# zdebruine/singlet

Hardware: AMD Instinct MI355X
Metric: ALS iterations/sec (1M cells x 30k genes, 5% nnz, k=50) (higher is better)
Workload: dtype f64

## Files before the change

singlet_amd/csrc/kernels_tiled.hip:

```cpp
#include "sgl_internal.h"
#include <atomic>
#include <hipcub/hipcub.hpp>
#include <stdlib.h>
#include <utility>
#include <type_traits>

#define TILED_NW 8
#define TILED_CW 64
#define TILED_NP 32
#define TILED_LDS_BYTES (160 * 1024 - 512)
#define TILED_SLACK 4096

__device__ __forceinline__ int64_t tiled_slot_col(const int32_t* __restrict__ perm, int64_t ncol, int64_t wb, int h, int p, int nsl) {
    const int64_t pos = wb * (TILED_NP * nsl) + nsl * p + h;
    if (pos >= ncol) return -1;
    return perm ? (int64_t)perm[pos] : pos;
}

__global__ void tiled_count_kernel(const int64_t* __restrict__ seg, const int32_t* __restrict__ perm, int64_t ncol, int T, int64_t nwb,
                                   uint8_t* __restrict__ cnt, int64_t* __restrict__ chunk_entries, int nsl) {
    const int64_t u = (int64_t)blockIdx.x * blockDim.x + threadIdx.x;
    if (u >= nwb * T) return;
    const int64_t wb = u / T;
    const int t = (int)(u - wb * T);
    int64_t tot = 0;
    for (int p = 0; p < TILED_NP; ++p) {
        int64_t n = 0;
        for (int h = 0; h < nsl; ++h) {
            const int64_t col = tiled_slot_col(perm, ncol, wb, h, p, nsl);
            if (col >= 0) {
                const int64_t c = seg[(int64_t)(t + 1) * ncol + col] - seg[(int64_t)t * ncol + col];
                n = c > n ? c : n;
            }
        }
        int g = (int)((n + 3) >> 2);
        const int gps = 16 / nsl;
        if (p == TILED_NP - 1) g += (int)((gps - ((tot + g) & (gps - 1))) & (gps - 1));
        cnt[u * TILED_NP + p] = (uint8_t)g;
        tot += g;
    }
    chunk_entries[u] = tot * 4 * nsl;
}

__global__ __launch_bounds__(256) void tiled_fill_kernel(const double* __restrict__ x, const int32_t* __restrict__ idx,
                                                         const int64_t* __restrict__ seg, const int32_t* __restrict__ perm,
                                                         int64_t ncol, int T, int64_t nwb, int TR, int row_bytes,
                                                         const uint8_t* __restrict__ cnt,
                                                         const int64_t* __restrict__ cstart,
                                                         uint32_t* __restrict__ sroff, double* __restrict__ sx,
                                                         int masked, uint64_t seed, SglDiv inv_density, int mask_t,
                                                         int64_t col_off, int64_t row_off, int nsl) {
    const int lane = threadIdx.x & 63;
    const int eps = 64 / nsl, eps_sh = nsl == 4 ? 4 : 5;
    const int64_t gw = ((int64_t)blockIdx.x * blockDim.x + threadIdx.x) >> 6;
    const int64_t nw = ((int64_t)gridDim.x * blockDim.x) >> 6;
    for (int64_t u = gw; u < nwb * T; u += nw) {
        const int64_t wb = u / T;
        const int t = (int)(u - wb * T);
        const int64_t c0 = cstart[u];
        int P = 0;
        for (int p = 0; p < TILED_NP; ++p) {
            const int n4 = 4 * (int)cnt[u * TILED_NP + p];
            if (n4 == 0) continue;
            for (int h = 0; h < nsl; ++h) {
                const int64_t col = tiled_slot_col(perm, ncol, wb, h, p, nsl);
                int64_t a = 0, b = 0;
                if (col >= 0) { a = seg[(int64_t)t * ncol + col]; b = seg[(int64_t)(t + 1) * ncol + col]; }
                for (int q = lane; q < n4; q += 64) {
                    uint32_t ro = 0;
                    double xv = 0.0;
                    if (a + q < b) {
                        const int32_t r = idx[a + q];
                        ro = (uint32_t)(r - t * TR) * (uint32_t)row_bytes;
                        xv = x[a + q];
                        if (masked) {
                            const uint64_t gc = (uint64_t)(col + col_off), gr = (uint64_t)(r + row_off);
                            if (mask_t ? sgl_draw(seed, gr, gc, inv_density) : sgl_draw(seed, gc, gr, inv_density)) xv = 0.0;
                        }
                    }
                    const int pos = P + q;
                    const int64_t dst = c0 + (int64_t)(pos >> eps_sh) * 64 + h * eps + (pos & (eps - 1));
                    if (sroff != nullptr) sroff[dst] = ro;
                    sx[dst] = xv;
                }
            }
            P += n4;
        }
    }
// ... 34 lines not shown
    *p = nullptr;
    *cap = 0;
    const size_t want = count + count / 32 + 64;
    SGLCHK(t_alloc(p, want));
    *cap = want;
    return SGL_OK;
}

void sgl_tiled_free(DevTiled& S) {
    if (S.seg) (void)sgl_pool_free(S.seg);
    if (S.perm) (void)sgl_pool_free(S.perm);
    if (S.roff) (void)sgl_pool_free(S.roff);
    if (S.x) (void)sgl_pool_free(S.x);
    if (S.cstart) (void)sgl_pool_free(S.cstart);
    if (S.cnt) (void)sgl_pool_free(S.cnt);
    if (S.gtab) (void)sgl_pool_free(S.gtab);
    if (S.part) (void)sgl_pool_free(S.part);
    if (S.xm) (void)sgl_pool_free(S.xm);
    S = DevTiled();
}

static bool tiled_sort_columns() {
    const char* e = getenv("SGL_TILED_SORT");
    return !(e && *e == '0');
}

__global__ void tiled_col_keys_kernel(const int64_t* __restrict__ p, int64_t ncol, uint32_t* __restrict__ keys, int32_t* __restrict__ iota) {
    for (int64_t c = (int64_t)blockIdx.x * blockDim.x + threadIdx.x; c < ncol; c += (int64_t)gridDim.x * blockDim.x) {
        keys[c] = (uint32_t)(p[c + 1] - p[c]);
        iota[c] = (int32_t)c;
// ... 59 lines not shown
    S.KS = KS;
    int TR = TILED_LDS_BYTES / (KS * 8);
    TR = TR / 8 * 8;
    if (TR > 984) TR = 984;
    if (TR < 8 || k > 64) { sgl_set_error("tiled accumulate: k=%d unsupported", k); return SGL_EINVAL; }
    S.nwb = ((int64_t)M.ncol + S.CW - 1) / S.CW;
    {
        const int64_t groups = (S.nwb + TILED_NW - 1) / TILED_NW, T0 = ((int64_t)M.nrow + TR - 1) / TR;
        if (groups * T0 < 256 && !getenv("SGL_TILED_FULL_TILES")) {
            const int64_t want = std::min<int64_t>((256 + groups - 1) / groups, ((int64_t)M.nrow + 127) / 128);
            if (want > T0) TR = std::min<int>(TR, (int)(((((int64_t)M.nrow + want - 1) / want) + 7) / 8 * 8));
        }
    }
    S.TR = TR;
    S.T = (int)((M.nrow + TR - 1) / TR);
    S.ncol = M.ncol;
    S.nrow = M.nrow;
    S.src_nnz = M.nnz;
    const int64_t nchunks = S.nwb * S.T;

    int rc = SGL_OK;
    if (!tiled_sort_columns()) {
        if (S.perm) { (void)sgl_pool_free(S.perm); S.perm = nullptr; S.cap_perm = 0; }
    } else if (!S.perm || S.perm_nnz != M.nnz || S.cap_perm < (size_t)M.ncol) {
        rc = tiled_build_perm(c, M, S);
    }
    sgl_trace_setup("  stream: column order");
    if (rc == SGL_OK) rc = t_reserve(&S.seg, &S.cap_seg, (size_t)(S.T + 1) * (size_t)M.ncol);
    sgl_trace_setup("  stream: segment buffer reserved");
    DevCSC tmp = M;
    tmp.tile_rows = TR;
    tmp.ntiles = S.T;
    tmp.seg = S.seg;
    if (rc == SGL_OK) rc = k_build_segments(s, tmp);
    int64_t* chunk_entries = nullptr;
    if (rc == SGL_OK) rc = t_alloc(&chunk_entries, (size_t)nchunks);
    if (rc == SGL_OK) rc = t_reserve(&S.cnt, &S.cap_cnt, (size_t)nchunks * TILED_NP);
    if (rc == SGL_OK) rc = t_reserve(&S.cstart, &S.cap_cstart, (size_t)nchunks + 1);
    if (rc == SGL_OK) {
        tiled_count_kernel<<<dim3((unsigned)((nchunks + 255) / 256)), dim3(256), 0, s>>>(S.seg, S.perm, M.ncol, S.T, S.nwb, S.cnt,
                                                                                         chunk_entries, nsl);
        if (hipGetLastError() != hipSuccess) { sgl_set_error("tiled build: count kernel launch failed"); rc = SGL_EHIP; }
    }
    if (rc == SGL_OK) rc = k_exclusive_scan(c, chunk_entries, S.cstart, nchunks);
    if (rc == SGL_OK) rc = k_scan_total(s, chunk_entries, S.cstart, nchunks);
    int64_t E = 0;
    if (rc == SGL_OK) {
        if (hipMemcpyAsync(&E, S.cstart + nchunks, sizeof(int64_t), hipMemcpyDeviceToHost, s) != hipSuccess ||
            hipStreamSynchronize(s) != hipSuccess) { sgl_set_error("tiled build: reading the stream size failed"); rc = SGL_EHIP; }
    }
    S.E = E;
    sgl_trace_setup("  stream: segments, counts, scan");
    if (rc == SGL_OK) rc = t_reserve(&S.roff, &S.cap_roff, (size_t)E + TILED_SLACK);
    if (rc == SGL_OK) rc = t_reserve(&S.x, &S.cap_x, (size_t)E + TILED_SLACK);
    sgl_trace_setup("  stream: roff / x buffers reserved");
    if (rc == SGL_OK) {
        if (hipMemsetAsync(S.roff + E, 0, TILED_SLACK * sizeof(uint32_t), s) != hipSuccess ||
            hipMemsetAsync(S.x + E, 0, TILED_SLACK * sizeof(double), s) != hipSuccess) { sgl_set_error("tiled build: clearing the stream slack failed"); rc = SGL_EHIP; }
    }
    if (rc == SGL_OK && nchunks > 0) {
        int64_t blocks = (nchunks + 3) / 4;
        if (blocks > 256 * 64) blocks = 256 * 64;
        tiled_fill_kernel<<<dim3((unsigned)blocks), dim3(256), 0, s>>>(M.x, M.i, S.seg, S.perm, M.ncol, S.T, S.nwb, TR, KS * 8,
                                                                       S.cnt, S.cstart, S.roff, S.x, 0, 0, sgl_div_make(1), 0, 0, 0, nsl);
        if (hipGetLastError() != hipSuccess) { sgl_set_error("tiled build: fill kernel launch failed"); rc = SGL_EHIP; }
    }
    const size_t ngroups = (size_t)(E / (4 * nsl));
    if (rc == SGL_OK) rc = t_reserve(&S.gtab, &S.cap_gtab, ngroups + 256);
    if (rc == SGL_OK) {
        if (hipMemsetAsync(S.gtab + ngroups, 0, 256 * sizeof(uint16_t), s) != hipSuccess) { sgl_set_error("tiled build: clearing the schedule slack failed"); rc = SGL_EHIP; }
    }
    if (rc == SGL_OK && nchunks > 0) {
        int64_t blocks = (nchunks + 3) / 4;
        if (blocks > 256 * 64) blocks = 256 * 64;
        tiled_gtab_kernel<<<dim3((unsigned)blocks), dim3(256), 0, s>>>(S.cnt, S.cstart, nchunks, nsl, S.gtab);
        if (hipGetLastError() != hipSuccess) { sgl_set_error("tiled build: schedule kernel launch failed"); rc = SGL_EHIP; }
    }
    const int64_t nwg_x = (S.nwb + TILED_NW - 1) / TILED_NW;
    int R = 1;
    const int r_fill = nwg_x < 1024 ? (int)std::max<int64_t>(1, (512 + nwg_x - 1) / nwg_x) : 1;
    const double top_share = nsl == 4 ? S.top_share4 : S.top_share;
    const bool skewed = S.perm && top_share * (double)nwg_x > 1.5;
    const int r_bal = skewed ? (int)std::min<double>(256.0, ceil(top_share * 256.0 / 0.35)) : 1;
    if (r_bal > r_fill) {
        double best = -1.0;
        const int rmin = std::max(r_fill, (int)std::min<int64_t>(r_bal, std::max(1, S.T)));
        if (rmin > S.T) R = std::max(1, S.T);
        for (int r = rmin; r <= std::min<int64_t>(S.T, rmin + rmin / 4 + 4); ++r) {
            const int tpr = (S.T + r - 1) / r;
            const int reff = (S.T + tpr - 1) / tpr;
            const double wgs = (double)nwg_x * reff;
            const double eff = wgs / (ceil(wgs / 256.0) * 256.0);
            if (eff > best + 1e-9) { best = eff; R = reff; }
        }
    } else if (r_fill > 1 && S.T > 1 && !getenv("SGL_TILED_OLD_SPLIT")) {
        const double t_tile = (double)E / (double)nsl / ((double)nwg_x * (double)S.T) * 2.4e-9 + 2.5e-6;
        const double t_wg = 6e-6;
        double best = 1e300;
        for (int r = 1; r <= std::min<int64_t>(S.T, 64); ++r) {
            const double wgs = (double)nwg_x * r;
            const double rounds = ceil(wgs / 256.0);
            const int largest = (S.T + r - 1) / r;
            const double cost = rounds * ((double)largest * t_tile + t_wg) + (r > 1 ? (double)r * (double)k * (double)M.ncol * 16.0 / 4e12 : 0.0);
            if (cost < best * (1.0 - 1e-9)) { best = cost; R = r; }
        }
    } else if (r_fill > 1 && getenv("SGL_TILED_OLD_SPLIT")) {
        double best = -1.0;
        for (int r = r_fill; r <= std::min<int64_t>(S.T, 4 * r_fill); ++r) {
            const int tpr = (S.T + r - 1) / r;
            const int reff = (S.T + tpr - 1) / tpr;
            const double wgs = (double)nwg_x * reff;
            const double eff = wgs / (ceil(wgs / 256.0) * 256.0);
            if (eff > best + 1e-9) { best = eff; R = reff; }
        }
    }
    if (const char* fr = getenv("SGL_TILED_RANGES")) {
        if (atoi(fr) > 0) R = atoi(fr);
    }
    S.range_fastest = r_bal > r_fill;
    S.R = std::max(1, std::min(R, std::max(1, S.T)));
    S.tiles_per_range = (S.T + S.R - 1) / S.R;
    S.tail_wg0 = -1;
    S.tail_R = 1;
    if (S.R == 1 && !S.range_fastest && nwg_x > 256 && S.T > 1 && E >= (4ll << 20) && !getenv("SGL_TILED_NO_TAIL")) {
        const int64_t tail = nwg_x % 256;
        if (tail > 0) {
            const double t_tile = (double)E / (double)nsl / ((double)nwg_x * (double)S.T) * 2.4e-9 + 2.5e-6;
            const double t_wg = 6e-6;
            const double tail_cols = (double)tail * TILED_NW * S.CW;
            double best = (double)S.T * t_tile + t_wg;
            int Rt = 1;
            for (int r = 2; r <= std::min<int64_t>(S.T, 16); ++r) {
                const double rounds = ceil((double)tail * r / 256.0);
                const double cost = rounds * ((double)((S.T + r - 1) / r) * t_tile + t_wg) + (double)r * (double)k * tail_cols * 16.0 / 4e12;
                if (cost < best * (1.0 - 1e-9)) { best = cost; Rt = r; }
            }
            if (Rt > 1) { S.tail_wg0 = nwg_x - tail; S.tail_R = Rt; }
        }
    }
    if (rc == SGL_OK && S.R > 1) rc = t_reserve(&S.part, &S.cap_part, (size_t)S.R * (size_t)k * (size_t)M.ncol);
    if (rc == SGL_OK && S.tail_R > 1)
        rc = t_reserve(&S.part, &S.cap_part, (size_t)S.tail_R * (size_t)k * (size_t)((nwg_x - S.tail_wg0) * TILED_NW * S.CW));
    hipError_t e = hipStreamSynchronize(s);
    if (chunk_entries) (void)sgl_pool_free(chunk_entries);
    if (rc == SGL_OK && e != hipSuccess) { sgl_set_error("tiled build failed: %s", hipGetErrorString(e)); rc = SGL_EHIP; }
    if (rc != SGL_OK) { sgl_tiled_free(S); return rc; }
    S.built = true;
    ++S.builds;
    return rc;
}

int sgl_tiled_mask_values(sgl_ctx* c, const DevCSC& M, DevTiled& S, uint64_t seed, uint64_t inv_density, int mask_t,
                          int64_t col_off, int64_t row_off) {
    if (!S.built || !S.seg) { sgl_set_error("masked values: no entry stream"); return SGL_ESTATE; }
    if (S.xm && S.xm_seed == seed && S.xm_inv == inv_density && S.xm_mask_t == mask_t) return SGL_OK;
    hipStream_t s = c->stream;
    S.xm_mask_t = -1;
    SGLCHK(t_reserve(&S.xm, &S.cap_xm, (size_t)S.E + TILED_SLACK));
    HIPCHK(hipMemsetAsync(S.xm + S.E, 0, TILED_SLACK * sizeof(double), s));
    const int64_t nchunks = S.nwb * S.T;
    if (nchunks > 0) {
        const int KS = S.KS;
        int64_t blocks = (nchunks + 3) / 4;
        if (blocks > 256 * 64) blocks = 256 * 64;
        tiled_fill_kernel<<<dim3((unsigned)blocks), dim3(256), 0, s>>>(M.x, M.i, S.seg, S.perm, M.ncol, S.T, S.nwb, S.TR, KS * 8, S.cnt,
                                                                       S.cstart, nullptr, S.xm, 1, seed, sgl_div_make(inv_density),
                                                                       mask_t, col_off, row_off, S.NSL);
        HIPCHK(hipGetLastError());
    }
    S.xm_seed = seed; S.xm_inv = inv_density; S.xm_mask_t = mask_t;
    return SGL_OK;
}


__device__ __forceinline__ void acc_load(int idx4, double& v0, double& v1) {
    int a, b, c, d;
    asm volatile(
        "s_set_gpr_idx_on %4, gpr_idx(SRC0)\n\tv_mov_b32 %0, v128\n\tv_mov_b32 %1, v129\n\tv_mov_b32 %2, v130\n\t"
        "v_mov_b32 %3, v131\n\ts_set_gpr_idx_off"
        : "=v"(a), "=v"(b), "=v"(c), "=v"(d) : "s"(idx4) : "memory");
    v0 = __hiloint2double(b, a);
    v1 = __hiloint2double(d, c);
}

#include "acc_tiled_gen.inc"

template <int MODE>
__global__ __launch_bounds__(512) __attribute__((amdgpu_waves_per_eu(8, 8))) void acc_tiled_kernel(
    const uint32_t* __restrict__ sroff, const double* __restrict__ sx, const int64_t* __restrict__ cstart,
    const uint8_t* __restrict__ cnt, int T, int64_t nwb, const double* __restrict__ F, int k, int TR, int64_t nrow,
    int tiles_per_range, double* __restrict__ Bout, int64_t ncol, int KS, int ldf, int ldb, int64_t slab,
    const int32_t* __restrict__ perm, int range_fastest, const uint16_t* __restrict__ gtab, int tail_wg0, int tail_R,
    double* __restrict__ tail_part, int64_t tail_slab) {
    constexpr int NSL = (MODE == 4 || MODE == 7) ? 4 : 2;
    constexpr bool PAIRRING = MODE == 3 || MODE == 6;
    asm volatile("" ::: "v255");
    extern __shared__ __attribute__((aligned(16))) char smem[];
    double* tile = reinterpret_cast<double*>(smem);
    const int lane = threadIdx.x & 63;
    const int wave = __builtin_amdgcn_readfirstlane((int)(threadIdx.x >> 6));
    unsigned bx = blockIdx.x, by = blockIdx.y;
    if (range_fastest) {
        const unsigned unit = blockIdx.x + gridDim.x * blockIdx.y, nranges = gridDim.y;
        bx = unit / nranges;
        by = unit - bx * nranges;
    }
    unsigned nry = gridDim.y;
    bool tail_piece = false;
    if (tail_R > 1 && (int)bx >= tail_wg0) {
        const unsigned u = bx - (unsigned)tail_wg0;
        bx = (unsigned)tail_wg0 + u / (unsigned)tail_R;
        by = u % (unsigned)tail_R;
        nry = (unsigned)tail_R;
        tail_piece = true;
    }
    const int64_t wb = (int64_t)bx * TILED_NW + wave;
    const int t0 = (int)(((int64_t)by * T) / nry);
    const int t1 = (int)((((int64_t)by + 1) * T) / nry);
    const bool wact = wb < nwb;
    typedef __attribute__((address_space(3))) char lds_char;
    constexpr int LMASK = NSL == 4 ? 15 : 31;
    const unsigned lane16 = (unsigned)(uintptr_t)(lds_char*)smem + (lane & LMASK) * 16;
    const unsigned slot = PAIRRING ? (unsigned)((lane >> 5) * 32 + (lane & 15)) : (unsigned)lane;
    const unsigned voff4 = slot * 4, voff8 = slot * 8;
    constexpr unsigned LAP_R = (NSL == 4 ? 256u : 128u) * 8u;
    const unsigned pfl = (unsigned)lane * (LAP_R / 64u) + (unsigned)ACC_TILED_PF_LAPS * LAP_R;

    asm volatile(ACC_TILED_ZERO_ASM ::: "memory");

    uint64_t rp = 0, xp = 0;
    int phase = 0;
    uint64_t qn0 = 0, qn1 = 0, qn2 = 0, qn3 = 0;
    int64_t pos_next = 0;
    if (wact) {
        const int64_t pos = cstart[wb * T + t0];
        pos_next = cstart[wb * T + t0 + 1];
        const uint64_t* cq = reinterpret_cast<const uint64_t*>(cnt + (wb * T + t0) * TILED_NP);
        qn0 = cq[0]; qn1 = cq[1]; qn2 = cq[2]; qn3 = cq[3];
        const uint64_t r_ = reinterpret_cast<uint64_t>(sroff + pos), x_ = reinterpret_cast<uint64_t>(sx + pos);
        rp = ((uint64_t)(uint32_t)__builtin_amdgcn_readfirstlane((unsigned)(r_ >> 32)) << 32) | (uint32_t)__builtin_amdgcn_readfirstlane((unsigned)r_);
        xp = ((uint64_t)(uint32_t)__builtin_amdgcn_readfirstlane((unsigned)(x_ >> 32)) << 32) | (uint32_t)__builtin_amdgcn_readfirstlane((unsigned)x_);
        if constexpr (NSL == 4)
            asm volatile(ACC_TILED4_RING_FILL_ASM : [rp] "+s"(rp), [xp] "+s"(xp) : [voff4] "v"(voff4), [voff8] "v"(voff8) : ACC_TILED_CLOBBERS);
        else if constexpr (PAIRRING)
            asm volatile(ACC_TILED2R_RING_FILL_ASM : [rp] "+s"(rp), [xp] "+s"(xp) : [voff4] "v"(voff4), [voff8] "v"(voff8) : ACC_TILED_CLOBBERS);
        else
            asm volatile(ACC_TILED_RING_FILL_ASM : [rp] "+s"(rp), [xp] "+s"(xp) : [voff4] "v"(voff4), [voff8] "v"(voff8) : ACC_TILED_CLOBBERS);
    }
    if constexpr (NSL == 4) {
        for (int e = (int)threadIdx.x; e < TILED_LDS_BYTES / 8; e += 64 * TILED_NW) tile[e] = 0.0;
    }

    int64_t pos_cur = wact ? cstart[wb * T + t0] : 0;
    for (int t = t0; t < t1; ++t) {
        const uint64_t q0 = qn0, q1 = qn1, q2 = qn2, q3 = qn3;
        const int nsets = (int)((pos_next - pos_cur) >> 6);
        const int64_t pos_chunk = pos_cur;
        pos_cur = pos_next;
        if (wact && t + 1 < t1) {
            const uint64_t* cq = reinterpret_cast<const uint64_t*>(cnt + (wb * T + t + 1) * TILED_NP);
            qn0 = cq[0]; qn1 = cq[1]; qn2 = cq[2]; qn3 = cq[3];
            pos_next = cstart[wb * T + t + 2];
        }

        const int64_t row0 = (int64_t)t * TR;
        const int rows = (int)((nrow - row0 < TR) ? (nrow - row0) : TR);
        const int n = rows * k;
        const double* __restrict__ src = F + row0 * ldf;
        if constexpr (NSL == 4) {
            const int c16 = (int)threadIdx.x & 15, r0 = (int)threadIdx.x >> 4;
            constexpr int RPR = 64 * TILED_NW / 16;
            const bool vec = ((k | ldf) & 1) == 0 && (reinterpret_cast<uintptr_t>(src) & 15) == 0;
            if (vec) {
                constexpr int RST = 4;
                double2 stg[RST];
                const bool cact = 2 * c16 < k;
#pragma unroll
                for (int j = 0; j < RST; ++j) {
                    const int r = r0 + j * RPR;
                    stg[j] = double2{0.0, 0.0};
                    if (cact && r < rows) stg[j] = *reinterpret_cast<const double2*>(src + (int64_t)r * ldf + 2 * c16);
                }
                __syncthreads();
                for (int rb = 0; rb < rows; rb += RST * RPR) {
#pragma unroll
                    for (int j = 0; j < RST; ++j) {
                        const int r = rb + r0 + j * RPR;
                        if (cact && r < rows) *reinterpret_cast<double2*>(tile + r * 32 + 2 * c16) = stg[j];
                    }
                    if (rb + RST * RPR < rows) {
#pragma unroll
                        for (int j = 0; j < RST; ++j) {
                            const int r = rb + RST * RPR + r0 + j * RPR;
                            stg[j] = double2{0.0, 0.0};
                            if (cact && r < rows) stg[j] = *reinterpret_cast<const double2*>(src + (int64_t)r * ldf + 2 * c16);
                        }
                    }
                }
            } else {
                __syncthreads();
                for (int r = r0; r < rows; r += RPR) {
                    if (c16 < k) tile[r * 32 + c16] = src[(int64_t)r * ldf + c16];
                    if (c16 + 16 < k) tile[r * 32 + c16 + 16] = src[(int64_t)r * ldf + c16 + 16];
                }
            }
        } else if (KS == k && ldf == k) {
            constexpr int RST = 8;
            constexpr int NRND = (TILED_LDS_BYTES / 16 + RST * 64 * TILED_NW - 1) / (RST * 64 * TILED_NW);
            static_assert(NRND * RST * 64 * TILED_NW * 16 >= TILED_LDS_BYTES, "staging must cover the whole tile");
            double2 stg[RST];
#pragma unroll
            for (int j = 0; j < RST; ++j) {
                const int e = ((int)threadIdx.x + j * 64 * TILED_NW) * 2;
                stg[j] = double2{0.0, 0.0};
                if (e < n) stg[j] = *reinterpret_cast<const double2*>(src + e);
            }
            __syncthreads();
#pragma unroll
            for (int rd = 0; rd < NRND; ++rd) {
#pragma unroll
                for (int j = 0; j < RST; ++j) {
                    const int e = ((int)threadIdx.x + (rd * RST + j) * 64 * TILED_NW) * 2;
                    if (e < n) *reinterpret_cast<double2*>(tile + e) = stg[j];
                }
                if (rd + 1 < NRND) {
#pragma unroll
                    for (int j = 0; j < RST; ++j) {
                        const int e = ((int)threadIdx.x + ((rd + 1) * RST + j) * 64 * TILED_NW) * 2;
                        stg[j] = double2{0.0, 0.0};
                        if (e < n) stg[j] = *reinterpret_cast<const double2*>(src + e);
                    }
                }
            }
        } else {
            __syncthreads();
            if (((k | ldf) & 1) == 0 && (reinterpret_cast<uintptr_t>(src) & 15) == 0) {
                const int hp = k >> 1;
                for (int e = (int)threadIdx.x; e < rows * hp; e += 64 * TILED_NW) {
                    const int r = e / hp, c2 = (e - r * hp) * 2;
                    *reinterpret_cast<double2*>(tile + r * KS + c2) = *reinterpret_cast<const double2*>(src + (int64_t)r * ldf + c2);
                }
            } else {
                for (int e = (int)threadIdx.x; e < n; e += 64 * TILED_NW) {
                    const int r = e / k, f = e - r * k;
                    tile[r * KS + f] = src[(int64_t)r * ldf + f];
                }
            }
            if (KS != k)
                for (int r = (int)threadIdx.x; r < rows; r += 64 * TILED_NW) tile[r * KS + k] = 0.0;
        }
        __builtin_amdgcn_s_waitcnt(0x0F70);
        __syncthreads();
        if (wact && nsets > 0) {
            if constexpr (MODE == 6 || MODE == 7) {
                const uint64_t t_ = reinterpret_cast<uint64_t>(gtab + pos_chunk / (4 * NSL));
                const uint64_t tp = ((uint64_t)(uint32_t)__builtin_amdgcn_readfirstlane((unsigned)(t_ >> 32)) << 32) | (uint32_t)__builtin_amdgcn_readfirstlane((unsigned)t_);
                if constexpr (MODE == 6)
                    asm volatile(ACC_TILED2T_CHUNK_ASM
                                 : [rp] "+s"(rp), [xp] "+s"(xp), [phase] "+s"(phase)
                                 : [ns] "s"(2 * nsets), [tp] "s"(tp), [lane16] "v"(lane16), [voff4] "v"(voff4), [voff8] "v"(voff8), [pfl] "v"(pfl)
                                 : ACC_TILEDT_CLOBBERS);
                else
                    asm volatile(ACC_TILED4T_CHUNK_ASM
                                 : [rp] "+s"(rp), [xp] "+s"(xp), [phase] "+s"(phase)
                                 : [ns] "s"(nsets), [tp] "s"(tp), [lane16] "v"(lane16), [voff4] "v"(voff4), [voff8] "v"(voff8), [pfl] "v"(pfl)
                                 : ACC_TILEDT_CLOBBERS);
            } else if constexpr (MODE == 4)
// ... 87 lines not shown
                                   hipFuncAttributeMaxDynamicSharedMemorySize, TILED_LDS_BYTES + 512));
        if (dev >= 0 && dev < 64) attr_set[dev] = true;
    }
    const int64_t nwg_x = (S.nwb + TILED_NW - 1) / TILED_NW;
    const bool slabs = S.R > 1;
    double* out = slabs ? S.part : B;
    const int64_t n = (int64_t)kf * S.ncol;
    const bool tail = !slabs && S.tail_R > 1 && S.tail_wg0 >= 0;
    const int64_t tail_cols = tail ? (nwg_x - S.tail_wg0) * TILED_NW * S.CW : 0;
    const int64_t tail_slab = tail_cols * kf;
    const dim3 grid(tail ? (unsigned)(S.tail_wg0 + (nwg_x - S.tail_wg0) * S.tail_R) : (unsigned)nwg_x, (unsigned)S.R);
    const bool table = !getenv("SGL_TILED_NO_TABLE") && !getenv("SGL_TILED_PREP") && S.gtab != nullptr;
    auto launch = [&](auto mode) {
        constexpr int MODE = decltype(mode)::value;
        acc_tiled_kernel<MODE><<<grid, dim3(64 * TILED_NW), lds, s>>>(
            S.roff, xvals ? xvals : S.x, S.cstart, S.cnt, S.T, S.nwb, F, kf, S.TR, S.nrow, S.tiles_per_range, out, S.ncol, KS, ldf,
            slabs ? kf : ldb, slabs ? n : 0, S.perm, S.range_fastest ? 1 : 0, S.gtab, tail ? (int)S.tail_wg0 : -1, tail ? S.tail_R : 1,
            S.part, tail_slab);
    };
    if (S.NSL == 4 && table) launch(std::integral_constant<int, 7>());
    else if (S.NSL == 2 && table) launch(std::integral_constant<int, 6>());
    else if (S.NSL == 4) launch(std::integral_constant<int, 4>());
    else if (!getenv("SGL_TILED_PREP")) launch(std::integral_constant<int, 3>());
    else launch(std::integral_constant<int, 2>());
    HIPCHK(hipGetLastError());
    if (tail) {
        const int64_t pos0 = S.tail_wg0 * TILED_NW * S.CW;
        const int64_t ne = (S.ncol - pos0) * kf;
        if (ne > 0) {
            int64_t blocks = (ne + 255) / 256;
            if (blocks > 4096) blocks = 4096;
// ... 30 lines not shown
```

singlet_amd/csrc/sgl_internal.h:

```cpp
#pragma once
#include <hip/hip_runtime.h>
#include <stdint.h>
#include <stdio.h>
#include <stdarg.h>
#include <vector>
#include <algorithm>

#include "../../include/singlet_hip.h"

#define SGL_WAVE 64
#define SGL_MAX_K 1024
#define SGL_LANE_NNLS_MAX_K 128

void sgl_set_error(const char* fmt, ...);

hipError_t sgl_pool_malloc_raw(void** p, size_t bytes);
template <typename T_>
inline hipError_t sgl_pool_malloc(T_** p, size_t bytes) { return sgl_pool_malloc_raw(reinterpret_cast<void**>(p), bytes); }
hipError_t sgl_pool_free(void* p);
hipError_t sgl_pool_mem_info(size_t* free_b, size_t* total_b);
void sgl_pool_release(void);
size_t sgl_pool_cached_bytes(void);

#define HIPCHK(expr)                                                                                   \
// ... 14 lines not shown
struct DevCSC {
    double* x = nullptr;
    int32_t* i = nullptr;
    int64_t* p = nullptr;
    int32_t nrow = 0, ncol = 0;
    int64_t nnz = 0;
    int64_t* seg = nullptr;
    int32_t tile_rows = 0, ntiles = 0;
};

struct DevTiled {
    uint32_t* roff = nullptr;
    double* x = nullptr;
    int64_t* cstart = nullptr;
    uint8_t* cnt = nullptr;
    uint16_t* gtab = nullptr;
    size_t cap_gtab = 0;
    double* part = nullptr;
    double* xm = nullptr;
    uint64_t xm_seed = 0, xm_inv = 0;
    int xm_mask_t = -1;
    int64_t* seg = nullptr;
    int32_t* perm = nullptr;
    size_t cap_perm = 0;
    int64_t perm_nnz = -1;
    bool range_fastest = false;
    double top_share = 0.0;
    double top_share4 = 0.0;
    size_t cap_roff = 0, cap_x = 0, cap_cstart = 0, cap_cnt = 0, cap_part = 0, cap_xm = 0, cap_seg = 0;
    bool built = false;
    int64_t builds = 0;
    int64_t src_nnz = -1;
    int32_t TR = 0, T = 0, CW = 0, k = 0, R = 1, tiles_per_range = 0;
    int64_t tail_wg0 = -1;
    int32_t tail_R = 1;
    int32_t NSL = 2;
    int32_t KS = 0;
    int64_t nwb = 0, E = 0, ncol = 0, nrow = 0;
};

struct PhaseEvent {
    int phase;
    hipEvent_t e0, e1;
};

struct NnlsPass {
    const int32_t* list;
    const uint32_t* count;
// ... 290 lines not shown
```

Measured before the change: 39.70.

## Split row tiles into double-buffered half-blocks with lookahead padding redistribution

Row tiles are split into half-tiles of D=TR/2 rows, and the LDS factor tile becomes a two-slot ring, so the next half-block can be staged while the current one is processed. This removes the full-tile reload and barrier between tiles. The count kernel now runs one wave per column block and redistributes each chunk's padding into entries from the following half-block, recording per-slot offsets in a new 'ahead' array. This is meant to cut padded zero entries in the stream. It adds a more complex build step, an extra metadata buffer, and moves the range/tail split decision to before the build using an estimated entry count.

```diff
diff --git a/singlet_amd/csrc/kernels_tiled.hip b/singlet_amd/csrc/kernels_tiled.hip
--- a/singlet_amd/csrc/kernels_tiled.hip
+++ b/singlet_amd/csrc/kernels_tiled.hip
@@ -17,36 +17,77 @@
     return perm ? (int64_t)perm[pos] : pos;
 }
 
-__global__ void tiled_count_kernel(const int64_t* __restrict__ seg, const int32_t* __restrict__ perm, int64_t ncol, int T, int64_t nwb,
-                                   uint8_t* __restrict__ cnt, int64_t* __restrict__ chunk_entries, int nsl) {
-    const int64_t u = (int64_t)blockIdx.x * blockDim.x + threadIdx.x;
-    if (u >= nwb * T) return;
-    const int64_t wb = u / T;
-    const int t = (int)(u - wb * T);
-    int64_t tot = 0;
-    for (int p = 0; p < TILED_NP; ++p) {
-        int64_t n = 0;
-        for (int h = 0; h < nsl; ++h) {
-            const int64_t col = tiled_slot_col(perm, ncol, wb, h, p, nsl);
-            if (col >= 0) {
-                const int64_t c = seg[(int64_t)(t + 1) * ncol + col] - seg[(int64_t)t * ncol + col];
-                n = c > n ? c : n;
-            }
-        }
-        int g = (int)((n + 3) >> 2);
-        const int gps = 16 / nsl;
-        if (p == TILED_NP - 1) g += (int)((gps - ((tot + g) & (gps - 1))) & (gps - 1));
-        cnt[u * TILED_NP + p] = (uint8_t)g;
-        tot += g;
-    }
-    chunk_entries[u] = tot * 4 * nsl;
+__device__ __forceinline__ int tiled_ranges_of(int64_t wb, int R, int64_t tail_wg0, int tail_R) {
+    return (tail_R > 1 && tail_wg0 >= 0 && wb / TILED_NW >= tail_wg0) ? tail_R : R;
+}
+__device__ __forceinline__ int tiled_range_end(int b, int T, int NB, int nr) {
+    const int t = b >> 1;
+    const int y = (int)(((int64_t)(t + 1) * nr - 1) / T);
+    const int b1 = 2 * (int)(((int64_t)(y + 1) * T) / nr);
+    return b1 < NB ? b1 : NB;
+}
+
+__global__ __launch_bounds__(256) void tiled_count_kernel(const int64_t* __restrict__ seg, const int32_t* __restrict__ perm, int64_t ncol,
+                                                          int T, int NB, int64_t nwb, int R, int64_t tail_wg0, int tail_R,
+                                                          uint8_t* __restrict__ cnt, uint16_t* __restrict__ ahead,
+                                                          int64_t* __restrict__ chunk_entries, int nsl) {
+    const int lane = threadIdx.x & 63, p = lane & 31;
+    const int64_t wb = ((int64_t)blockIdx.x * blockDim.x + threadIdx.x) >> 6;
+    if (wb >= nwb) return;
+    const int gps = 16 / nsl;
+    int64_t col[4];
+    for (int h = 0; h < 4; ++h) col[h] = h < nsl ? tiled_slot_col(perm, ncol, wb, h, p, nsl) : -1;
+    const int nr = tiled_ranges_of(wb, R, tail_wg0, tail_R);
+    for (int b0 = 0; b0 < NB;) {
+        const int b1 = tiled_range_end(b0, T, NB, nr);
+        int64_t pos[4];
+        for (int h = 0; h < 4; ++h) pos[h] = col[h] >= 0 ? seg[(int64_t)b0 * ncol + col[h]] : 0;
+        for (int b = b0; b < b1; ++b) {
+            const int hi = b + 2 < b1 ? b + 2 : b1;
+            int64_t must = 0, avail = 0, ew[4];
+            for (int h = 0; h < 4; ++h) {
+                ew[h] = 0;
+                if (col[h] >= 0) {
+                    const int64_t eb = seg[(int64_t)(b + 1) * ncol + col[h]];
+                    ew[h] = seg[(int64_t)hi * ncol + col[h]];
+                    must = eb - pos[h] > must ? eb - pos[h] : must;
+                    avail = ew[h] - pos[h] > avail ? ew[h] - pos[h] : avail;
+                }
+            }
+            int g = (int)((must + 3) >> 2);
+            const int cap = (int)((avail + 3) >> 2) - g;
+            int tot = g;
+            for (int o = 16; o > 0; o >>= 1) tot += __shfl_xor(tot, o, 32);
+            const int rem = (gps - (tot & (gps - 1))) & (gps - 1);
+            int suf = cap;
+            for (int o = 1; o < 32; o <<= 1) {
+                const int v = __shfl_down(suf, o, 32);
+                if (p + o < 32) suf += v;
+            }
+            const int above = suf - cap;
+            int extra = rem - above < cap ? rem - above : cap;
+            if (extra < 0) extra = 0;
+            const int all = __shfl(suf, 0, 32);
+            if (p == TILED_NP - 1 && rem > all) extra += rem - all;
+            g += extra;
+            const int64_t u = wb * NB + b;
+            if (lane < 32) {
+                cnt[u * TILED_NP + p] = (uint8_t)g;
+                for (int h = 0; h < nsl; ++h)
+                    ahead[u * (TILED_NP * nsl) + nsl * p + h] = col[h] >= 0 ? (uint16_t)(pos[h] - seg[(int64_t)b * ncol + col[h]]) : (uint16_t)0;
+            }
+            if (lane == 0) chunk_entries[u] = (int64_t)(tot + rem) * 4 * nsl;
+            for (int h = 0; h < 4; ++h) pos[h] += (4 * (int64_t)g < ew[h] - pos[h]) ? 4 * (int64_t)g : ew[h] - pos[h];
+        }
+        b0 = b1;
+    }
 }
 
 __global__ __launch_bounds__(256) void tiled_fill_kernel(const double* __restrict__ x, const int32_t* __restrict__ idx,
                                                          const int64_t* __restrict__ seg, const int32_t* __restrict__ perm,
-                                                         int64_t ncol, int T, int64_t nwb, int TR, int row_bytes,
-                                                         const uint8_t* __restrict__ cnt,
-                                                         const int64_t* __restrict__ cstart,
+                                                         int64_t ncol, int T, int NB, int64_t nwb, int R, int64_t tail_wg0, int tail_R,
+                                                         int D, int row_bytes, const uint8_t* __restrict__ cnt,
+                                                         const uint16_t* __restrict__ ahead, const int64_t* __restrict__ cstart,
                                                          uint32_t* __restrict__ sroff, double* __restrict__ sx,
                                                          int masked, uint64_t seed, SglDiv inv_density, int mask_t,
                                                          int64_t col_off, int64_t row_off, int nsl) {
@@ -54,9 +95,11 @@
     const int eps = 64 / nsl, eps_sh = nsl == 4 ? 4 : 5;
     const int64_t gw = ((int64_t)blockIdx.x * blockDim.x + threadIdx.x) >> 6;
     const int64_t nw = ((int64_t)gridDim.x * blockDim.x) >> 6;
-    for (int64_t u = gw; u < nwb * T; u += nw) {
-        const int64_t wb = u / T;
-        const int t = (int)(u - wb * T);
+    for (int64_t u = gw; u < nwb * NB; u += nw) {
+        const int64_t wb = u / NB;
+        const int b = (int)(u - wb * NB);
+        const int b1 = tiled_range_end(b, T, NB, tiled_ranges_of(wb, R, tail_wg0, tail_R));
+        const int hi = b + 2 < b1 ? b + 2 : b1;
         const int64_t c0 = cstart[u];
         int P = 0;
         for (int p = 0; p < TILED_NP; ++p) {
@@ -64,14 +107,18 @@
             if (n4 == 0) continue;
             for (int h = 0; h < nsl; ++h) {
                 const int64_t col = tiled_slot_col(perm, ncol, wb, h, p, nsl);
-                int64_t a = 0, b = 0;
-                if (col >= 0) { a = seg[(int64_t)t * ncol + col]; b = seg[(int64_t)(t + 1) * ncol + col]; }
+                int64_t a = 0, e = 0;
+                if (col >= 0) {
+                    a = seg[(int64_t)b * ncol + col] + ahead[u * (TILED_NP * nsl) + nsl * p + h];
+                    e = seg[(int64_t)hi * ncol + col];
+                }
                 for (int q = lane; q < n4; q += 64) {
                     uint32_t ro = 0;
                     double xv = 0.0;
-                    if (a + q < b) {
+                    if (a + q < e) {
                         const int32_t r = idx[a + q];
-                        ro = (uint32_t)(r - t * TR) * (uint32_t)row_bytes;
+                        const int blk = r >= (b + 1) * D ? b + 1 : b;
+                        ro = (uint32_t)((blk & 1) * D + (r - blk * D)) * (uint32_t)row_bytes;
                         xv = x[a + q];
                         if (masked) {
                             const uint64_t gc = (uint64_t)(col + col_off), gr = (uint64_t)(r + row_off);
@@ -136,6 +183,7 @@
     if (S.x) (void)sgl_pool_free(S.x);
     if (S.cstart) (void)sgl_pool_free(S.cstart);
     if (S.cnt) (void)sgl_pool_free(S.cnt);
+    if (S.ahead) (void)sgl_pool_free(S.ahead);
     if (S.gtab) (void)sgl_pool_free(S.gtab);
     if (S.part) (void)sgl_pool_free(S.part);
     if (S.xm) (void)sgl_pool_free(S.xm);
@@ -225,10 +273,12 @@
     }
     S.TR = TR;
     S.T = (int)((M.nrow + TR - 1) / TR);
+    const int D = TR / 2;
+    S.NB = (int)((M.nrow + D - 1) / D);
     S.ncol = M.ncol;
     S.nrow = M.nrow;
     S.src_nnz = M.nnz;
-    const int64_t nchunks = S.nwb * S.T;
+    const int64_t nchunks = S.nwb * S.NB;
 
     int rc = SGL_OK;
     if (!tiled_sort_columns()) {
@@ -237,56 +287,7 @@
         rc = tiled_build_perm(c, M, S);
     }
     sgl_trace_setup("  stream: column order");
-    if (rc == SGL_OK) rc = t_reserve(&S.seg, &S.cap_seg, (size_t)(S.T + 1) * (size_t)M.ncol);
-    sgl_trace_setup("  stream: segment buffer reserved");
-    DevCSC tmp = M;
-    tmp.tile_rows = TR;
-    tmp.ntiles = S.T;
-    tmp.seg = S.seg;
-    if (rc == SGL_OK) rc = k_build_segments(s, tmp);
-    int64_t* chunk_entries = nullptr;
-    if (rc == SGL_OK) rc = t_alloc(&chunk_entries, (size_t)nchunks);
-    if (rc == SGL_OK) rc = t_reserve(&S.cnt, &S.cap_cnt, (size_t)nchunks * TILED_NP);
-    if (rc == SGL_OK) rc = t_reserve(&S.cstart, &S.cap_cstart, (size_t)nchunks + 1);
-    if (rc == SGL_OK) {
-        tiled_count_kernel<<<dim3((unsigned)((nchunks + 255) / 256)), dim3(256), 0, s>>>(S.seg, S.perm, M.ncol, S.T, S.nwb, S.cnt,
-                                                                                         chunk_entries, nsl);
-        if (hipGetLastError() != hipSuccess) { sgl_set_error("tiled build: count kernel launch failed"); rc = SGL_EHIP; }
-    }
-    if (rc == SGL_OK) rc = k_exclusive_scan(c, chunk_entries, S.cstart, nchunks);
-    if (rc == SGL_OK) rc = k_scan_total(s, chunk_entries, S.cstart, nchunks);
-    int64_t E = 0;
-    if (rc == SGL_OK) {
-        if (hipMemcpyAsync(&E, S.cstart + nchunks, sizeof(int64_t), hipMemcpyDeviceToHost, s) != hipSuccess ||
-            hipStreamSynchronize(s) != hipSuccess) { sgl_set_error("tiled build: reading the stream size failed"); rc = SGL_EHIP; }
-    }
-    S.E = E;
-    sgl_trace_setup("  stream: segments, counts, scan");
-    if (rc == SGL_OK) rc = t_reserve(&S.roff, &S.cap_roff, (size_t)E + TILED_SLACK);
-    if (rc == SGL_OK) rc = t_reserve(&S.x, &S.cap_x, (size_t)E + TILED_SLACK);
-    sgl_trace_setup("  stream: roff / x buffers reserved");
-    if (rc == SGL_OK) {
-        if (hipMemsetAsync(S.roff + E, 0, TILED_SLACK * sizeof(uint32_t), s) != hipSuccess ||
-            hipMemsetAsync(S.x + E, 0, TILED_SLACK * sizeof(double), s) != hipSuccess) { sgl_set_error("tiled build: clearing the stream slack failed"); rc = SGL_EHIP; }
-    }
-    if (rc == SGL_OK && nchunks > 0) {
-        int64_t blocks = (nchunks + 3) / 4;
-        if (blocks > 256 * 64) blocks = 256 * 64;
-        tiled_fill_kernel<<<dim3((unsigned)blocks), dim3(256), 0, s>>>(M.x, M.i, S.seg, S.perm, M.ncol, S.T, S.nwb, TR, KS * 8,
-                                                                       S.cnt, S.cstart, S.roff, S.x, 0, 0, sgl_div_make(1), 0, 0, 0, nsl);
-        if (hipGetLastError() != hipSuccess) { sgl_set_error("tiled build: fill kernel launch failed"); rc = SGL_EHIP; }
-    }
-    const size_t ngroups = (size_t)(E / (4 * nsl));
-    if (rc == SGL_OK) rc = t_reserve(&S.gtab, &S.cap_gtab, ngroups + 256);
-    if (rc == SGL_OK) {
-        if (hipMemsetAsync(S.gtab + ngroups, 0, 256 * sizeof(uint16_t), s) != hipSuccess) { sgl_set_error("tiled build: clearing the schedule slack failed"); rc = SGL_EHIP; }
-    }
-    if (rc == SGL_OK && nchunks > 0) {
-        int64_t blocks = (nchunks + 3) / 4;
-        if (blocks > 256 * 64) blocks = 256 * 64;
-        tiled_gtab_kernel<<<dim3((unsigned)blocks), dim3(256), 0, s>>>(S.cnt, S.cstart, nchunks, nsl, S.gtab);
-        if (hipGetLastError() != hipSuccess) { sgl_set_error("tiled build: schedule kernel launch failed"); rc = SGL_EHIP; }
-    }
+    const double E_est = (double)M.nnz * 1.06;
     const int64_t nwg_x = (S.nwb + TILED_NW - 1) / TILED_NW;
     int R = 1;
     const int r_fill = nwg_x < 1024 ? (int)std::max<int64_t>(1, (512 + nwg_x - 1) / nwg_x) : 1;
@@ -305,7 +306,7 @@
             if (eff > best + 1e-9) { best = eff; R = reff; }
         }
     } else if (r_fill > 1 && S.T > 1 && !getenv("SGL_TILED_OLD_SPLIT")) {
-        const double t_tile = (double)E / (double)nsl / ((double)nwg_x * (double)S.T) * 2.4e-9 + 2.5e-6;
+        const double t_tile = E_est / (double)nsl / ((double)nwg_x * (double)S.T) * 2.4e-9 + 2.5e-6;
         const double t_wg = 6e-6;
         double best = 1e300;
         for (int r = 1; r <= std::min<int64_t>(S.T, 64); ++r) {
@@ -333,10 +334,10 @@
     S.tiles_per_range = (S.T + S.R - 1) / S.R;
     S.tail_wg0 = -1;
     S.tail_R = 1;
-    if (S.R == 1 && !S.range_fastest && nwg_x > 256 && S.T > 1 && E >= (4ll << 20) && !getenv("SGL_TILED_NO_TAIL")) {
+    if (S.R == 1 && !S.range_fastest && nwg_x > 256 && S.T > 1 && E_est >= (double)(4ll << 20) && !getenv("SGL_TILED_NO_TAIL")) {
         const int64_t tail = nwg_x % 256;
         if (tail > 0) {
-            const double t_tile = (double)E / (double)nsl / ((double)nwg_x * (double)S.T) * 2.4e-9 + 2.5e-6;
+            const double t_tile = E_est / (double)nsl / ((double)nwg_x * (double)S.T) * 2.4e-9 + 2.5e-6;
             const double t_wg = 6e-6;
             const double tail_cols = (double)tail * TILED_NW * S.CW;
             double best = (double)S.T * t_tile + t_wg;
@@ -348,6 +349,58 @@
             }
             if (Rt > 1) { S.tail_wg0 = nwg_x - tail; S.tail_R = Rt; }
         }
+    }
+    if (rc == SGL_OK) rc = t_reserve(&S.seg, &S.cap_seg, (size_t)(S.NB + 1) * (size_t)M.ncol);
+    sgl_trace_setup("  stream: segment buffer reserved");
+    DevCSC tmp = M;
+    tmp.tile_rows = D;
+    tmp.ntiles = S.NB;
+    tmp.seg = S.seg;
+    if (rc == SGL_OK) rc = k_build_segments(s, tmp);
+    int64_t* chunk_entries = nullptr;
+    if (rc == SGL_OK) rc = t_alloc(&chunk_entries, (size_t)nchunks);
+    if (rc == SGL_OK) rc = t_reserve(&S.cnt, &S.cap_cnt, (size_t)nchunks * TILED_NP);
+    if (rc == SGL_OK) rc = t_reserve(&S.ahead, &S.cap_ahead, (size_t)nchunks * (size_t)S.CW);
+    if (rc == SGL_OK) rc = t_reserve(&S.cstart, &S.cap_cstart, (size_t)nchunks + 1);
+    if (rc == SGL_OK && S.nwb > 0) {
+        tiled_count_kernel<<<dim3((unsigned)((S.nwb + 3) / 4)), dim3(256), 0, s>>>(S.seg, S.perm, M.ncol, S.T, S.NB, S.nwb, S.R,
+                                                                                   S.tail_wg0, S.tail_R, S.cnt, S.ahead, chunk_entries, nsl);
+        if (hipGetLastError() != hipSuccess) { sgl_set_error("tiled build: count kernel launch failed"); rc = SGL_EHIP; }
+    }
+    if (rc == SGL_OK) rc = k_exclusive_scan(c, chunk_entries, S.cstart, nchunks);
+    if (rc == SGL_OK) rc = k_scan_total(s, chunk_entries, S.cstart, nchunks);
+    int64_t E = 0;
+    if (rc == SGL_OK) {
+        if (hipMemcpyAsync(&E, S.cstart + nchunks, sizeof(int64_t), hipMemcpyDeviceToHost, s) != hipSuccess ||
+            hipStreamSynchronize(s) != hipSuccess) { sgl_set_error("tiled build: reading the stream size failed"); rc = SGL_EHIP; }
+    }
+    S.E = E;
+    sgl_trace_setup("  stream: segments, counts, scan");
+    if (rc == SGL_OK) rc = t_reserve(&S.roff, &S.cap_roff, (size_t)E + TILED_SLACK);
+    if (rc == SGL_OK) rc = t_reserve(&S.x, &S.cap_x, (size_t)E + TILED_SLACK);
+    sgl_trace_setup("  stream: roff / x buffers reserved");
+    if (rc == SGL_OK) {
+        if (hipMemsetAsync(S.roff + E, 0, TILED_SLACK * sizeof(uint32_t), s) != hipSuccess ||
+            hipMemsetAsync(S.x + E, 0, TILED_SLACK * sizeof(double), s) != hipSuccess) { sgl_set_error("tiled build: clearing the stream slack failed"); rc = SGL_EHIP; }
+    }
+    if (rc == SGL_OK && nchunks > 0) {
+        int64_t blocks = (nchunks + 3) / 4;
+        if (blocks > 256 * 64) blocks = 256 * 64;
+        tiled_fill_kernel<<<dim3((unsigned)blocks), dim3(256), 0, s>>>(M.x, M.i, S.seg, S.perm, M.ncol, S.T, S.NB, S.nwb, S.R, S.tail_wg0,
+                                                                       S.tail_R, D, KS * 8, S.cnt, S.ahead, S.cstart, S.roff, S.x,
+                                                                       0, 0, sgl_div_make(1), 0, 0, 0, nsl);
+        if (hipGetLastError() != hipSuccess) { sgl_set_error("tiled build: fill kernel launch failed"); rc = SGL_EHIP; }
+    }
+    const size_t ngroups = (size_t)(E / (4 * nsl));
+    if (rc == SGL_OK) rc = t_reserve(&S.gtab, &S.cap_gtab, ngroups + 256);
+    if (rc == SGL_OK) {
+        if (hipMemsetAsync(S.gtab + ngroups, 0, 256 * sizeof(uint16_t), s) != hipSuccess) { sgl_set_error("tiled build: clearing the schedule slack failed"); rc = SGL_EHIP; }
+    }
+    if (rc == SGL_OK && nchunks > 0) {
+        int64_t blocks = (nchunks + 3) / 4;
+        if (blocks > 256 * 64) blocks = 256 * 64;
+        tiled_gtab_kernel<<<dim3((unsigned)blocks), dim3(256), 0, s>>>(S.cnt, S.cstart, nchunks, nsl, S.gtab);
+        if (hipGetLastError() != hipSuccess) { sgl_set_error("tiled build: schedule kernel launch failed"); rc = SGL_EHIP; }
     }
     if (rc == SGL_OK && S.R > 1) rc = t_reserve(&S.part, &S.cap_part, (size_t)S.R * (size_t)k * (size_t)M.ncol);
     if (rc == SGL_OK && S.tail_R > 1)
@@ -363,20 +416,20 @@
 
 int sgl_tiled_mask_values(sgl_ctx* c, const DevCSC& M, DevTiled& S, uint64_t seed, uint64_t inv_density, int mask_t,
                           int64_t col_off, int64_t row_off) {
-    if (!S.built || !S.seg) { sgl_set_error("masked values: no entry stream"); return SGL_ESTATE; }
+    if (!S.built || !S.seg || !S.ahead) { sgl_set_error("masked values: no entry stream"); return SGL_ESTATE; }
     if (S.xm && S.xm_seed == seed && S.xm_inv == inv_density && S.xm_mask_t == mask_t) return SGL_OK;
     hipStream_t s = c->stream;
     S.xm_mask_t = -1;
     SGLCHK(t_reserve(&S.xm, &S.cap_xm, (size_t)S.E + TILED_SLACK));
     HIPCHK(hipMemsetAsync(S.xm + S.E, 0, TILED_SLACK * sizeof(double), s));
-    const int64_t nchunks = S.nwb * S.T;
+    const int64_t nchunks = S.nwb * S.NB;
     if (nchunks > 0) {
         const int KS = S.KS;
         int64_t blocks = (nchunks + 3) / 4;
         if (blocks > 256 * 64) blocks = 256 * 64;
-        tiled_fill_kernel<<<dim3((unsigned)blocks), dim3(256), 0, s>>>(M.x, M.i, S.seg, S.perm, M.ncol, S.T, S.nwb, S.TR, KS * 8, S.cnt,
-                                                                       S.cstart, nullptr, S.xm, 1, seed, sgl_div_make(inv_density),
-                                                                       mask_t, col_off, row_off, S.NSL);
+        tiled_fill_kernel<<<dim3((unsigned)blocks), dim3(256), 0, s>>>(M.x, M.i, S.seg, S.perm, M.ncol, S.T, S.NB, S.nwb, S.R, S.tail_wg0,
+                                                                       S.tail_R, S.TR / 2, KS * 8, S.cnt, S.ahead, S.cstart, nullptr, S.xm,
+                                                                       1, seed, sgl_div_make(inv_density), mask_t, col_off, row_off, S.NSL);
         HIPCHK(hipGetLastError());
     }
     S.xm_seed = seed; S.xm_inv = inv_density; S.xm_mask_t = mask_t;
@@ -396,10 +449,98 @@
 
 #include "acc_tiled_gen.inc"
 
+template <int NSL>
+__device__ __forceinline__ void tiled_stage(double* __restrict__ tile, const double* __restrict__ src, int rows, int k, int KS, int ldf,
+                                            bool sync) {
+    const int n = rows * k;
+    if constexpr (NSL == 4) {
+        const int c16 = (int)threadIdx.x & 15, r0 = (int)threadIdx.x >> 4;
+        constexpr int RPR = 64 * TILED_NW / 16;
+        const bool vec = ((k | ldf) & 1) == 0 && (reinterpret_cast<uintptr_t>(src) & 15) == 0;
+        if (vec) {
+            constexpr int RST = 4;
+            double2 stg[RST];
+            const bool cact = 2 * c16 < k;
+#pragma unroll
+            for (int j = 0; j < RST; ++j) {
+                const int r = r0 + j * RPR;
+                stg[j] = double2{0.0, 0.0};
+                if (cact && r < rows) stg[j] = *reinterpret_cast<const double2*>(src + (int64_t)r * ldf + 2 * c16);
+            }
+            if (sync) __syncthreads();
+            for (int rb = 0; rb < rows; rb += RST * RPR) {
+#pragma unroll
+                for (int j = 0; j < RST; ++j) {
+                    const int r = rb + r0 + j * RPR;
+                    if (cact && r < rows) *reinterpret_cast<double2*>(tile + r * 32 + 2 * c16) = stg[j];
+                }
+                if (rb + RST * RPR < rows) {
+#pragma unroll
+                    for (int j = 0; j < RST; ++j) {
+                        const int r = rb + RST * RPR + r0 + j * RPR;
+                        stg[j] = double2{0.0, 0.0};
+                        if (cact && r < rows) stg[j] = *reinterpret_cast<const double2*>(src + (int64_t)r * ldf + 2 * c16);
+                    }
+                }
+            }
+        } else {
+            if (sync) __syncthreads();
+            for (int r = r0; r < rows; r += RPR) {
+                if (c16 < k) tile[r * 32 + c16] = src[(int64_t)r * ldf + c16];
+                if (c16 + 16 < k) tile[r * 32 + c16 + 16] = src[(int64_t)r * ldf + c16 + 16];
+            }
+        }
+    } else if (KS == k && ldf == k) {
+        constexpr int RST = 8;
+        constexpr int NRND = (TILED_LDS_BYTES / 32 + RST * 64 * TILED_NW - 1) / (RST * 64 * TILED_NW);
+        static_assert(NRND * RST * 64 * TILED_NW * 16 >= TILED_LDS_BYTES / 2, "staging must cover a whole ring slot");
+        double2 stg[RST];
+#pragma unroll
+        for (int j = 0; j < RST; ++j) {
+            const int e = ((int)threadIdx.x + j * 64 * TILED_NW) * 2;
+            stg[j] = double2{0.0, 0.0};
+            if (e < n) stg[j] = *reinterpret_cast<const double2*>(src + e);
+        }
+        if (sync) __syncthreads();
+#pragma unroll
+        for (int rd = 0; rd < NRND; ++rd) {
+#pragma unroll
+            for (int j = 0; j < RST; ++j) {
+                const int e = ((int)threadIdx.x + (rd * RST + j) * 64 * TILED_NW) * 2;
+                if (e < n) *reinterpret_cast<double2*>(tile + e) = stg[j];
+            }
+            if (rd + 1 < NRND) {
+#pragma unroll
+                for (int j = 0; j < RST; ++j) {
+                    const int e = ((int)threadIdx.x + ((rd + 1) * RST + j) * 64 * TILED_NW) * 2;
+                    stg[j] = double2{0.0, 0.0};
+                    if (e < n) stg[j] = *reinterpret_cast<const double2*>(src + e);
+                }
+            }
+        }
+    } else {
+        if (sync) __syncthreads();
+        if (((k | ldf) & 1) == 0 && (reinterpret_cast<uintptr_t>(src) & 15) == 0) {
+            const int hp = k >> 1;
+            for (int e = (int)threadIdx.x; e < rows * hp; e += 64 * TILED_NW) {
+                const int r = e / hp, c2 = (e - r * hp) * 2;
+                *reinterpret_cast<double2*>(tile + r * KS + c2) = *reinterpret_cast<const double2*>(src + (int64_t)r * ldf + c2);
+            }
+        } else {
+            for (int e = (int)threadIdx.x; e < n; e += 64 * TILED_NW) {
+                const int r = e / k, f = e - r * k;
+                tile[r * KS + f] = src[(int64_t)r * ldf + f];
+            }
+        }
+        if (KS != k)
+            for (int r = (int)threadIdx.x; r < rows; r += 64 * TILED_NW) tile[r * KS + k] = 0.0;
+    }
+}
+
 template <int MODE>
 __global__ __launch_bounds__(512) __attribute__((amdgpu_waves_per_eu(8, 8))) void acc_tiled_kernel(
     const uint32_t* __restrict__ sroff, const double* __restrict__ sx, const int64_t* __restrict__ cstart,
-    const uint8_t* __restrict__ cnt, int T, int64_t nwb, const double* __restrict__ F, int k, int TR, int64_t nrow,
+    const uint8_t* __restrict__ cnt, int T, int NB, int64_t nwb, const double* __restrict__ F, int k, int TR, int64_t nrow,
     int tiles_per_range, double* __restrict__ Bout, int64_t ncol, int KS, int ldf, int ldb, int64_t slab,
     const int32_t* __restrict__ perm, int range_fastest, const uint16_t* __restrict__ gtab, int tail_wg0, int tail_R,
     double* __restrict__ tail_part, int64_t tail_slab) {
@@ -428,6 +569,8 @@
     const int64_t wb = (int64_t)bx * TILED_NW + wave;
     const int t0 = (int)(((int64_t)by * T) / nry);
     const int t1 = (int)((((int64_t)by + 1) * T) / nry);
+    const int D = TR >> 1;
+    const int b0 = 2 * t0, b1 = 2 * t1 < NB ? 2 * t1 : NB;
     const bool wact = wb < nwb;
     typedef __attribute__((address_space(3))) char lds_char;
     constexpr int LMASK = NSL == 4 ? 15 : 31;
@@ -444,9 +587,9 @@
     uint64_t qn0 = 0, qn1 = 0, qn2 = 0, qn3 = 0;
     int64_t pos_next = 0;
     if (wact) {
-        const int64_t pos = cstart[wb * T + t0];
-        pos_next = cstart[wb * T + t0 + 1];
-        const uint64_t* cq = reinterpret_cast<const uint64_t*>(cnt + (wb * T + t0) * TILED_NP);
+        const int64_t pos = cstart[wb * NB + b0];
+        pos_next = cstart[wb * NB + b0 + 1];
+        const uint64_t* cq = reinterpret_cast<const uint64_t*>(cnt + (wb * NB + b0) * TILED_NP);
         qn0 = cq[0]; qn1 = cq[1]; qn2 = cq[2]; qn3 = cq[3];
         const uint64_t r_ = reinterpret_cast<uint64_t>(sroff + pos), x_ = reinterpret_cast<uint64_t>(sx + pos);
         rp = ((uint64_t)(uint32_t)__builtin_amdgcn_readfirstlane((unsigned)(r_ >> 32)) << 32) | (uint32_t)__builtin_amdgcn_readfirstlane((unsigned)r_);
@@ -462,106 +605,27 @@
         for (int e = (int)threadIdx.x; e < TILED_LDS_BYTES / 8; e += 64 * TILED_NW) tile[e] = 0.0;
     }
 
-    int64_t pos_cur = wact ? cstart[wb * T + t0] : 0;
-    for (int t = t0; t < t1; ++t) {
+    int64_t pos_cur = wact ? cstart[wb * NB + b0] : 0;
+    for (int b = b0; b < b1; ++b) {
         const uint64_t q0 = qn0, q1 = qn1, q2 = qn2, q3 = qn3;
         const int nsets = (int)((pos_next - pos_cur) >> 6);
         const int64_t pos_chunk = pos_cur;
         pos_cur = pos_next;
-        if (wact && t + 1 < t1) {
-            const uint64_t* cq = reinterpret_cast<const uint64_t*>(cnt + (wb * T + t + 1) * TILED_NP);
+        if (wact && b + 1 < b1) {
+            const uint64_t* cq = reinterpret_cast<const uint64_t*>(cnt + (wb * NB + b + 1) * TILED_NP);
             qn0 = cq[0]; qn1 = cq[1]; qn2 = cq[2]; qn3 = cq[3];
-            pos_next = cstart[wb * T + t + 2];
-        }
-
-        const int64_t row0 = (int64_t)t * TR;
-        const int rows = (int)((nrow - row0 < TR) ? (nrow - row0) : TR);
-        const int n = rows * k;
-        const double* __restrict__ src = F + row0 * ldf;
-        if constexpr (NSL == 4) {
-            const int c16 = (int)threadIdx.x & 15, r0 = (int)threadIdx.x >> 4;
-            constexpr int RPR = 64 * TILED_NW / 16;
-            const bool vec = ((k | ldf) & 1) == 0 && (reinterpret_cast<uintptr_t>(src) & 15) == 0;
-            if (vec) {
-                constexpr int RST = 4;
-                double2 stg[RST];
-                const bool cact = 2 * c16 < k;
-#pragma unroll
-                for (int j = 0; j < RST; ++j) {
-                    const int r = r0 + j * RPR;
-                    stg[j] = double2{0.0, 0.0};
-                    if (cact && r < rows) stg[j] = *reinterpret_cast<const double2*>(src + (int64_t)r * ldf + 2 * c16);
-                }
-                __syncthreads();
-                for (int rb = 0; rb < rows; rb += RST * RPR) {
-#pragma unroll
-                    for (int j = 0; j < RST; ++j) {
-                        const int r = rb + r0 + j * RPR;
-                        if (cact && r < rows) *reinterpret_cast<double2*>(tile + r * 32 + 2 * c16) = stg[j];
-                    }
-                    if (rb + RST * RPR < rows) {
-#pragma unroll
-                        for (int j = 0; j < RST; ++j) {
-                            const int r = rb + RST * RPR + r0 + j * RPR;
-                            stg[j] = double2{0.0, 0.0};
-                            if (cact && r < rows) stg[j] = *reinterpret_cast<const double2*>(src + (int64_t)r * ldf + 2 * c16);
-                        }
-                    }
-                }
-            } else {
-                __syncthreads();
-                for (int r = r0; r < rows; r += RPR) {
-                    if (c16 < k) tile[r * 32 + c16] = src[(int64_t)r * ldf + c16];
-                    if (c16 + 16 < k) tile[r * 32 + c16 + 16] = src[(int64_t)r * ldf + c16 + 16];
-                }
-            }
-        } else if (KS == k && ldf == k) {
-            constexpr int RST = 8;
-            constexpr int NRND = (TILED_LDS_BYTES / 16 + RST * 64 * TILED_NW - 1) / (RST * 64 * TILED_NW);
-            static_assert(NRND * RST * 64 * TILED_NW * 16 >= TILED_LDS_BYTES, "staging must cover the whole tile");
-            double2 stg[RST];
-#pragma unroll
-            for (int j = 0; j < RST; ++j) {
-                const int e = ((int)threadIdx.x + j * 64 * TILED_NW) * 2;
-                stg[j] = double2{0.0, 0.0};
-                if (e < n) stg[j] = *reinterpret_cast<const double2*>(src + e);
-            }
+            pos_next = cstart[wb * NB + b + 2];
+        }
+
+#pragma clang loop unroll(disable)
+        for (int j = b == b0 ? b : b + 1; j <= b + 1 && j < b1; ++j) {
+            const int64_t row0 = (int64_t)j * D;
+            tiled_stage<NSL>(tile + (j & 1) * D * KS, F + row0 * ldf, (int)(nrow - row0 < D ? nrow - row0 : D), k, KS, ldf, j == b || b != b0);
+        }
+        if (b == b0 || b + 1 < b1) {
+            __builtin_amdgcn_s_waitcnt(0x0F70);
             __syncthreads();
-#pragma unroll
-            for (int rd = 0; rd < NRND; ++rd) {
-#pragma unroll
-                for (int j = 0; j < RST; ++j) {
-                    const int e = ((int)threadIdx.x + (rd * RST + j) * 64 * TILED_NW) * 2;
-                    if (e < n) *reinterpret_cast<double2*>(tile + e) = stg[j];
-                }
-                if (rd + 1 < NRND) {
-#pragma unroll
-                    for (int j = 0; j < RST; ++j) {
-                        const int e = ((int)threadIdx.x + ((rd + 1) * RST + j) * 64 * TILED_NW) * 2;
-                        stg[j] = double2{0.0, 0.0};
-                        if (e < n) stg[j] = *reinterpret_cast<const double2*>(src + e);
-                    }
-                }
-            }
-        } else {
-            __syncthreads();
-            if (((k | ldf) & 1) == 0 && (reinterpret_cast<uintptr_t>(src) & 15) == 0) {
-                const int hp = k >> 1;
-                for (int e = (int)threadIdx.x; e < rows * hp; e += 64 * TILED_NW) {
-                    const int r = e / hp, c2 = (e - r * hp) * 2;
-                    *reinterpret_cast<double2*>(tile + r * KS + c2) = *reinterpret_cast<const double2*>(src + (int64_t)r * ldf + c2);
-                }
-            } else {
-                for (int e = (int)threadIdx.x; e < n; e += 64 * TILED_NW) {
-                    const int r = e / k, f = e - r * k;
-                    tile[r * KS + f] = src[(int64_t)r * ldf + f];
-                }
-            }
-            if (KS != k)
-                for (int r = (int)threadIdx.x; r < rows; r += 64 * TILED_NW) tile[r * KS + k] = 0.0;
-        }
-        __builtin_amdgcn_s_waitcnt(0x0F70);
-        __syncthreads();
+        }
         if (wact && nsets > 0) {
             if constexpr (MODE == 6 || MODE == 7) {
                 const uint64_t t_ = reinterpret_cast<uint64_t>(gtab + pos_chunk / (4 * NSL));
@@ -679,7 +743,7 @@
     auto launch = [&](auto mode) {
         constexpr int MODE = decltype(mode)::value;
         acc_tiled_kernel<MODE><<<grid, dim3(64 * TILED_NW), lds, s>>>(
-            S.roff, xvals ? xvals : S.x, S.cstart, S.cnt, S.T, S.nwb, F, kf, S.TR, S.nrow, S.tiles_per_range, out, S.ncol, KS, ldf,
+            S.roff, xvals ? xvals : S.x, S.cstart, S.cnt, S.T, S.NB, S.nwb, F, kf, S.TR, S.nrow, S.tiles_per_range, out, S.ncol, KS, ldf,
             slabs ? kf : ldb, slabs ? n : 0, S.perm, S.range_fastest ? 1 : 0, S.gtab, tail ? (int)S.tail_wg0 : -1, tail ? S.tail_R : 1,
             S.part, tail_slab);
     };
diff --git a/singlet_amd/csrc/sgl_internal.h b/singlet_amd/csrc/sgl_internal.h
--- a/singlet_amd/csrc/sgl_internal.h
+++ b/singlet_amd/csrc/sgl_internal.h
@@ -52,6 +52,7 @@
     double* x = nullptr;
     int64_t* cstart = nullptr;
     uint8_t* cnt = nullptr;
+    uint16_t* ahead = nullptr;
     uint16_t* gtab = nullptr;
     size_t cap_gtab = 0;
     double* part = nullptr;
@@ -65,11 +66,12 @@
     bool range_fastest = false;
     double top_share = 0.0;
     double top_share4 = 0.0;
-    size_t cap_roff = 0, cap_x = 0, cap_cstart = 0, cap_cnt = 0, cap_part = 0, cap_xm = 0, cap_seg = 0;
+    size_t cap_roff = 0, cap_x = 0, cap_cstart = 0, cap_cnt = 0, cap_part = 0, cap_xm = 0, cap_seg = 0, cap_ahead = 0;
     bool built = false;
     int64_t builds = 0;
     int64_t src_nnz = -1;
     int32_t TR = 0, T = 0, CW = 0, k = 0, R = 1, tiles_per_range = 0;
+    int32_t NB = 0;
     int64_t tail_wg0 = -1;
     int32_t tail_R = 1;
     int32_t NSL = 2;
```

New measurement: 41.82 (median of 6 runs). 1.05x the previous value.
